# zdule/distributed_learning

Measured on AMD Instinct MI355X. Metric: images/sec (whole node) ResNet-50 synthetic ImageNet, higher is better.
Workload: dtype bf16

## Files before the change

csrc/include/dla_kernels.h:

```cpp
#pragma once

#include <hip/hip_runtime.h>
#include <stdint.h>

#include "dla_dtype.h"
#include "dla_lists.h"

namespace dla {

struct SgdParams {
  float lr;
  float momentum;
  float dampening;
  float weight_decay;
  float grad_scale;
  int nesterov;
  int first_step;
};

void launch_sgd_ema_list(const SgdList& list, const EmaSlots& ema, const float* omd, int nblocks, int grad_dtype,
                         bool use_momentum, const SgdParams& hp, hipStream_t stream);
void launch_ema_update_list(const EmaList& list, int nblocks, const float* omd, hipStream_t stream);
void launch_ema_swap_list(const EmaList& list, int nblocks, hipStream_t stream);
void launch_sgd_list(const SgdList& list, int nblocks, int grad_dtype, bool use_momentum, const SgdParams& hp,
// ... 120 lines not shown
                   int64_t M, int C, int dtype, const float* gamma, float* ws, float* part, float* dgamma,
                   float* dbeta, int mask_mode, hipStream_t stream, const float* ext_part = nullptr,
                   int ext_nrb = 0, int64_t ld_dy = 0);

constexpr int kMaxBnGroups = 4;
struct BnGroups {
  int n;
  int begin[kMaxBnGroups + 1];
  const uint16_t* x[kMaxBnGroups];
  uint16_t* y[kMaxBnGroups];
  const uint16_t* dy[kMaxBnGroups];
  int64_t ldy[kMaxBnGroups], lddy[kMaxBnGroups];
  int64_t ldx[kMaxBnGroups], lddx[kMaxBnGroups];
  int ldp[kMaxBnGroups];
  int C[kMaxBnGroups], tpr[kMaxBnGroups], nrb[kMaxBnGroups];
  const float* part[kMaxBnGroups];
  float* wpart[kMaxBnGroups];
  const float* gamma[kMaxBnGroups];
  const float* beta[kMaxBnGroups];
  float* rm[kMaxBnGroups];
  float* rv[kMaxBnGroups];
  float* ws[kMaxBnGroups];
  float eps[kMaxBnGroups], mom[kMaxBnGroups];
  uint16_t* dx[kMaxBnGroups];
  float* dgamma[kMaxBnGroups];
  float* dbeta[kMaxBnGroups];
};
int bn_group_bwd_rows(int64_t M, const int* C, int n);
void launch_bn_group_fwd(BnGroups G, int64_t M, hipStream_t stream);
void launch_bn_group_bwd(BnGroups G, bool ext, int64_t M, hipStream_t stream);

void launch_bn_relu_maxpool_fwd(const void* x, const float* ws, void* y, uint8_t* pos, int N, int H, int W, int C,
                                int OH, int OW, int k, int s, int p, hipStream_t stream);
void launch_bn_relu_maxpool_bwd(const void* dy_pool, const uint8_t* pos, const void* x, void* dx, int N, int H, int W,
                                int C, int OH, int OW, int k, int s, int p, const float* gamma, float* ws, float* part,
                                float* dgamma, float* dbeta, hipStream_t stream);

void launch_maxpool_fwd(const void* x, void* y, uint8_t* pos, int N, int H, int W, int C, int OH, int OW, int k,
                        int s, int p, int dtype, hipStream_t stream);
void launch_maxpool_bwd(const void* dy, const uint8_t* pos, void* dx, int N, int H, int W, int C, int OH, int OW,
                        int k, int s, int p, int dtype, hipStream_t stream);
bool pool_fast_index(int64_t work, int64_t d0, int64_t d1, int64_t d2);
void set_pool3_sep(int rows);
int pool3_strip_rows();
void launch_gap_fwd(const void* x, void* y, int N, int HW, int C, int dtype, hipStream_t stream);
void launch_subsample2(const void* x, void* y, int N, int H, int W, int C, hipStream_t stream);
void launch_gap_bwd(const void* dy, void* dx, int N, int HW, int C, int dtype, hipStream_t stream);

void set_mfma_pipeline(int p);
int mfma_pipeline();
int mfma_pipeline_for(int K);
enum TileCfg : int {
  kTileAuto = 0,
  kTile128x128 = 1,
  kTile128x64 = 2,
  kTile64x64 = 3,
  kTile256x128 = 4,
  kTile256x128w4 = 5,
  kTile128x256w4 = 6,
  kTile256x64 = 7,
  kTile256x256 = 8,
  kTile512x128 = 9
};
int pick_tile(int64_t M, int N, int tile, int K = 0, bool wide_ok = true, bool stats = false);
void set_tile256_min_k_stats(int k);
bool tile256_enabled();
bool tn256_enabled();
inline int tile_bm(int cfg) {
  if (cfg == kTile512x128) return 512;
  return cfg == kTile64x64 ? 64
                           : ((cfg == kTile256x128 || cfg == kTile256x128w4 || cfg == kTile256x64 || cfg == kTile256x256)
                                  ? 256
                                  : 128);
}
inline int tile_bn(int cfg) {
  if (cfg == kTile512x128) return 128;
  return (cfg == kTile128x256w4 || cfg == kTile256x256) ? 256
                                                       : ((cfg == kTile128x128 || cfg == kTile256x128 || cfg == kTile256x128w4) ? 128 : 64);
}
int gemm_nt_stats_rows(int M, int N, int tile = kTileAuto, int K = 0, bool stats_fwd = true);
void set_tile256_min_k(int k);
int gemm_stream_rows(int64_t M, int N, int K, int64_t lda, int64_t ldc, bool b_kmajor, bool add = false,
                     bool bnb = false);
struct BnBwdArgs;
bool launch_gemm_stream(const void* A, int64_t lda, const void* B, int64_t ldb, bool b_kmajor, void* C, int64_t ldc,
                        int M, int N, int K, float* stats, hipStream_t stream, const void* addend = nullptr,
                        int64_t ldd = 0, const uint8_t* addend_mask = nullptr, const BnBwdArgs* bn_bwd = nullptr,
                        const float* apply_ws = nullptr, void* apply_out = nullptr);
void set_gemm_stream(int mode);
bool gemm_direct_ok(int N, int64_t ldc, const void* addend, int64_t ldd);
void launch_gemm_direct(const void* A, int64_t lda, const void* B, int64_t ldb, bool b_kmajor, void* C, int64_t ldc,
                        int M, int N, int K, float* stats, const void* addend, int64_t ldd,
                        const uint8_t* addend_mask, hipStream_t stream);
void set_gemm_direct(int mode);
constexpr int kGemmApplyMaxK = 2048;
bool gemm_apply_ok(int64_t M, int N, int K);
void set_gemm_apply_max_k(int k);
void set_gemm256_direct(int mode);
bool gemm256_direct_enabled();
void set_wgrad_w4(int mode);
int gemm_apply_rows(int64_t M);
void launch_gemm_apply(const void* y, const void* r, const float* ws, const float* ws2, void* out, uint8_t* mask,
                       const void* B, int64_t ldb, void* C, int M, int N, int K, float* stats, hipStream_t stream,
                       void* xs = nullptr, int H = 0, int W = 0);
void set_gemm_persist(int blocks_per_cu);
bool conv_f32_supported(int C, int Cout, int64_t M, int K);
bool conv_f32_divisors_ok(int OH, int OW, int C, int S);
void set_conv_f32_buffers(int nb);
void launch_conv_f32_fwd(const float* x, int64_t ldx, int N, int H, int W, int C, const float* w, int Cout, int R,
                         int S, int pad, int stride, float* y, bool accumulate, hipStream_t st);
int conv_f32_wgrad_splits(int64_t M, int Cout, int K);
void launch_conv_f32_wgrad(const float* dy, const float* x, int64_t ldx, int N, int H, int W, int C, int Cout, int R,
                           int S, int pad, int stride, float* partial, int splits, float* dw, bool accumulate,
                           hipStream_t st);
struct BnBwdArgs {
  const void* x;
  const float* ws;
  const uint8_t* mask;
  int mode;
  float* part;
  int64_t ldx = 0;
};
void launch_gemm_nt(const void* A, int64_t lda, const void* B, int64_t ldb, void* C, int64_t ldc, int M, int N, int K,
                    float* stats, hipStream_t stream, const void* addend = nullptr, int64_t ld_addend = 0,
                    bool b_kmajor = false, int tile = kTileAuto, const BnBwdArgs* bn_bwd = nullptr,
                    const uint8_t* addend_mask = nullptr,
                    const void* addend2_s2 = nullptr, int H = 0, int W = 0);
int gemm_tn_splits(int Mo, int No, int K);
bool splitk_xcd_remap();
void set_tn256(int mode);
void set_splitk_blocks(int blocks);
int splitk_target_blocks();
void launch_gemm_tn(const void* A, int64_t lda, const void* B, int64_t ldb, float* partial, int splits, int Mo, int No,
                    int K, void* out, int out_dtype, float scale, bool accumulate, hipStream_t stream);
int conv1x1_dual_blocks(int64_t M, int Cin, int Cout);
int conv1x1_dual_groups(int64_t M, int Cin, int Cout);
bool conv1x1_dual_bn_ok(int64_t M, int Cin, int Cout);
bool launch_conv1x1_dual(const void* dy, const void* x, const void* w, void* dx, float* part, int64_t M, int Cin,
                         int Cout, hipStream_t stream, const void* ybn = nullptr, const uint8_t* mask = nullptr,
                         const float* ws = nullptr);
void launch_splitk_reduce(const float* partial, int splits, int64_t n, void* out, int out_dtype, float scale,
                          bool accumulate, hipStream_t stream, const void* addend = nullptr, int64_t ld_addend = 0,
                          int ncol = 1);
int gemm_nt_splitk_splits(int M, int N, int K);
void launch_gemm_nt_splitk(const void* A, int64_t lda, const void* B, int64_t ldb, bool b_kmajor, float* partial,
                           int splits, void* C, int M, int N, int K, const void* addend, int64_t ld_addend,
                           hipStream_t stream);

int conv3x3_stats_rows(int64_t P, int Cout, int tile = kTileAuto, int K = 0, bool wide_ok = true);
int pick_conv_tile(int64_t P, int N, int tile, int K, bool wide_ok);
bool halo_conv_eligible(int Cin, int Cout, int W, int stride, bool fwd);
void launch_conv3x3_halo(const void* x, const void* w, void* y, int N, int H, int W, float* stats,
                         hipStream_t stream, const void* addend = nullptr);
void launch_conv3x3_fwd(const void* x, const void* w, void* y, int N, int H, int W, int Cin, int Cout, int stride,
                        float* stats, hipStream_t stream, int tile = kTileAuto);
void launch_conv3x3_dgrad(const void* dy, const void* w, void* dx, int N, int H, int W, int Cin, int Cout,
                          const void* addend, hipStream_t stream, int tile = kTileAuto,
                          const BnBwdArgs* bn_bwd = nullptr);
void launch_conv3x3s2_dgrad(const void* dy, const void* w, void* dx, int N, int H, int W, int Cin, int Cout,
                            hipStream_t stream);
int stem_stats_rows(int64_t P, int Cout = 64);
int stem_stream_rows(int64_t P, int Cout);
bool launch_stem_stream(const void* xs, const void* wpk, void* y, int N, int BH, int BW, float* stats,
                        hipStream_t stream);
void set_stem_stream(int mode);

// ... 23 lines not shown
```

csrc/kernels/gemm_stream.hip:

```cpp
#include <cstdlib>

#include "dla_common.h"
#include "dla_kernels.h"
#include "dla_knob.h"
#include "dla_mfma.h"

namespace dla {

using namespace mm;

namespace {

constexpr int kSBM = 128;
constexpr int kChunkElems = kSBM * kBK;
__host__ __device__ constexpr int stream_lookahead(int KC, bool add) { return add ? 2 : 4; }

struct StreamArgs {
  const bf16_t* a;
  int64_t lda;
  const bf16_t* b;
  int64_t ldb;
  bf16_t* c;
  int64_t ldc;
  int M, N;
  int mg;
  int per_xcd;
  float* stats;
  const bf16_t* d;
  int64_t ldd;
  const uint8_t* dmask;
  const bf16_t* bx;
  int64_t ldbx;
  const float* bws;
  const uint8_t* bmask;
  int bmode;
  const float* aws;
  bf16_t* aout;
  int sBH, sBW;
  FastDiv sfW, sfH;
  uint32_t a_bytes;
};

__device__ __forceinline__ int perm64(int p) { return 16 * ((p >> 2) & 3) + 4 * (p >> 4) + (p & 3); }

__device__ __forceinline__ int img_off(int row, int lc) { return row * kBK + ((lc ^ ((row >> 1) & 7)) << 3); }

typedef int i32x4_t __attribute__((ext_vector_type(4)));


__host__ __device__ constexpr bool stream_two_blocks(bool add, bool bnb) { return add && !bnb; }

template <int BN, int KC, bool kBT, bool kStats, bool kAdd = false, int kBM = -1, bool kAp = false,
          bool kStem = false>
__global__ __launch_bounds__(256, stream_two_blocks(kAdd, kBM >= 0) ? 2 : 1) void gemm_stream_kernel(const StreamArgs s) {
  constexpr bool kBnb = kBM >= 0;
  static_assert(!kStem || (!kBT && !kAdd && !kBnb && !kAp && KC == 4), "stem: the K = 256 forward");
  static_assert(!kAp || (!kBT && !kAdd && !kBnb), "apply-on-load: forwards only");
  static_assert(!(kStats && kBnb), "the partials buffer holds either the statistics or the BN-backward sums");
  constexpr int kSP = stream_lookahead(KC, stream_two_blocks(kAdd, kBnb));
  constexpr int kSS = kSP + 1;
  constexpr int WN = 64;
  constexpr int WGN = BN / WN;
  constexpr int WGM = 4 / WGN;
  constexpr int WM = kSBM / WGM;
  constexpr int TJ = WM / 16;
  constexpr int Q = kSP / KC;
  static_assert(kSP % KC == 0, "the in-flight window must hold whole tiles");
  constexpr int D = kChunkElems / 8 / 256;
  constexpr int E = 2 * TJ;
  constexpr int F = (kAdd ? 3 * TJ : 0) + (kBnb ? (kBM == 2 ? 3 : 2) * TJ : 0);
  constexpr int kVmRaw = (kSP - 1) * (kAp ? 2 * D : D) + Q * (E + F);
  constexpr int kVmAfter = kVmRaw < 63 ? kVmRaw : 63;
  static_assert(kBnb || kVmRaw <= 63, "vmcnt is a 6-bit count");
  constexpr int kPanelElems = BN * kBK;

  extern __shared__ __attribute__((aligned(16))) char smem_raw[];
  bf16_t* Bs = reinterpret_cast<bf16_t*>(smem_raw);
  bf16_t* ring = Bs + KC * kPanelElems;
  float* coef = reinterpret_cast<float*>(ring + kSS * kChunkElems);

  const int tid = threadIdx.x, lane = tid & 63, wave = tid >> 6;
  const int wn = wave % WGN, wm = wave / WGN;
  const int lr = lane & 15, g = lane >> 4;
  const int nbn = s.N / BN;
  const int xcd = blockIdx.x & 7, slot = blockIdx.x >> 3;
  const int bn = slot % nbn;
  const int grp = xcd * s.per_xcd + slot / nbn;
  const int col0 = bn * BN;
  const int M = s.M;
  const int mt = (M + kSBM - 1) / kSBM;
  const int ntile = grp < mt ? (mt - grp + s.mg - 1) / s.mg : 0;
  const int nchunk = ntile * KC;

  {
    constexpr int kPer = BN * KC * kBK / 8 / 256;
    static_assert(BN * KC * kBK / 8 % 256 == 0, "whole chunks per thread");
    ushort8_t v[kPer];
#pragma unroll
    for (int u = 0; u < kPer; ++u) {
      const int c = tid + u * 256;
      if constexpr (!kBT) {
        const int n = c / (KC * 8), kc = c % (KC * 8);
        v[u] = *reinterpret_cast<const ushort8_t*>(s.b + (int64_t)(col0 + n) * s.ldb + kc * 8);
      } else {
        const int k = c / (BN / 8), nc = (c % (BN / 8)) * 8;
        v[u] = *reinterpret_cast<const ushort8_t*>(s.b + (int64_t)k * s.ldb + col0 + nc);
      }
    }
#pragma unroll
    for (int u = 0; u < kPer; ++u) {
      const int c = tid + u * 256;
      if constexpr (!kBT) {
        const int n = c / (KC * 8), kc = c % (KC * 8);
        const int row = (n & ~63) + perm64(n & 63);
        *reinterpret_cast<ushort8_t*>(Bs + (kc >> 3) * kPanelElems + img_off(row, kc & 7)) = v[u];
      } else {
        const int k = c / (BN / 8), nc = (c % (BN / 8)) * 8;
        bf16_t* sub = Bs + (k >> 6) * kPanelElems;
        const int kk = k & 63;
#pragma unroll
        for (int e = 0; e < 8; ++e) {
          const int n = nc + e, row = (n & ~63) + perm64(n & 63);
          sub[img_off(row, kk >> 3) + (kk & 7)] = v[u][e];
        }
      }
    }
  }

  const __amdgpu_buffer_rsrc_t ra = make_srd(s.a, kStem ? s.a_bytes : (uint32_t)((int64_t)M * s.lda * 2));
  int sbase[kStem ? D : 1];
  uint32_t smsk[kStem ? D : 1];
  const int stw = rm_glds_kc(tid) >> 4, shalf = rm_glds_kc(tid) & 8;
  uint32_t vo[D];
  int vr[D];
#pragma unroll
  for (int i = 0; i < D; ++i) {
    const int c = tid + i * 256, r = c >> 3;
    vr[i] = r;
    vo[i] = (uint32_t)(((int64_t)r * s.lda + rm_glds_kc(c)) * 2);
  }
  const uint32_t ring0 = lds_addr(ring) + (uint32_t)__builtin_amdgcn_readfirstlane(wave * 64 * 16);
  auto issue = [&](int q) {
    const int t = q / KC, kc = q % KC;
    const int64_t row0 = (int64_t)(grp + t * s.mg) * kSBM;
    uint32_t o[D];
    uint32_t soff;
    if constexpr (kStem) {
      if (kc == 0) {
#pragma unroll
        for (int i = 0; i < D; ++i) {
          const int64_t p = row0 + vr[i];
          smsk[i] = 0u;
          sbase[i] = 0;
          if (p < M) {
            const uint32_t q2 = fdiv((uint32_t)p, s.sfW);
            const int ow = (int)p - (int)q2 * s.sBW;
            const uint32_t nn = fdiv(q2, s.sfH);
            const int oh = (int)q2 - (int)nn * s.sBH;
            const int bw = ow - 2 + stw;
            if ((unsigned)bw < (unsigned)s.sBW) {
#pragma unroll
              for (int th = 0; th < 4; ++th) smsk[i] |= ((unsigned)(oh - 2 + th) < (unsigned)s.sBH) ? (1u << th) : 0u;
              sbase[i] = (((int)nn * s.sBH + oh - 2) * s.sBW + bw) * 16 + shalf;
            }
          }
        }
      }
#pragma unroll
      for (int i = 0; i < D; ++i)
        o[i] = ((smsk[i] >> kc) & 1u) ? (uint32_t)(sbase[i] + kc * s.sBW * 16) * 2u : kOOB;
      soff = 0u;
    } else {
#pragma unroll
      for (int i = 0; i < D; ++i) o[i] = row0 + vr[i] < M ? vo[i] : kOOB;
      soff = row0 < M ? (uint32_t)((row0 * s.lda + kc * kBK) * 2) : 0u;
    }
    bglds<D, 256 * 16>(o, ra, (uint32_t)__builtin_amdgcn_readfirstlane(soff),
                       ring0 + (uint32_t)((q % kSS) * kChunkElems * 2));
  };

  if constexpr (kAp) {
    for (int i = tid; i < 2 * KC * kBK; i += 256) coef[i] = s.aws[2 * KC * kBK + i];
  }
  asm volatile("s_waitcnt vmcnt(0) lgkmcnt(0)" ::: "memory");
  __syncthreads();

  const __amdgpu_buffer_rsrc_t rd = make_srd(kAdd ? (const void*)s.d : (const void*)s.c, kAdd ? (uint32_t)((int64_t)M * s.ldd * 2) : 0u);
  const __amdgpu_buffer_rsrc_t rmk =
      make_srd(kAdd && s.dmask ? (const void*)s.dmask : (const void*)s.c, kAdd && s.dmask ? (uint32_t)(((int64_t)M * s.ldd + 7) / 8) : 0u);
  i32x4_t dv[kAdd ? TJ : 1][2];
  uint32_t mb[kAdd ? TJ : 1];
  const __amdgpu_buffer_rsrc_t rbx = make_srd(kBnb ? (const void*)s.bx : (const void*)s.c,
                                              kBnb ? (uint32_t)((int64_t)M * s.ldbx * 2) : 0u);
  const __amdgpu_buffer_rsrc_t rbm = make_srd(kBM == 2 ? (const void*)s.bmask : (const void*)s.c,
                                              kBM == 2 ? (uint32_t)(((int64_t)M * s.ldc + 7) / 8) : 0u);
  i32x4_t xv[kBnb ? TJ : 1][2];
  uint32_t xb[kBM == 2 ? TJ : 1];
  float bmean[kBnb ? 16 : 1], bsc[kBM == 1 ? 16 : 1], bsh[kBM == 1 ? 16 : 1];
  if constexpr (kBnb) {
    const int gc = col0 + wn * WN + 16 * g;
#pragma unroll
    for (int e = 0; e < 16; ++e) {
      bmean[e] = s.bws[gc + e];
      if constexpr (kBM == 1) {
        bsc[e] = s.bws[2 * s.N + gc + e];
        bsh[e] = s.bws[3 * s.N + gc + e];
      }
    }
  }
  auto load_operands = [&](int t) {
    const int64_t row0 = (int64_t)(grp + t * s.mg) * kSBM;
    const int gc = col0 + wn * WN + 16 * g;
    if constexpr (kAdd) {
#pragma unroll
      for (int j = 0; j < TJ; ++j) {
        const int64_t gm = row0 + wm * WM + 16 * j + lr;
        const bool ok = gm < M;
        const uint32_t off = ok ? (uint32_t)((gm * s.ldd + gc) * 2) : kOOB;
        dv[j][0] = __builtin_amdgcn_raw_buffer_load_b128(rd, off, 0, 0);
        dv[j][1] = __builtin_amdgcn_raw_buffer_load_b128(rd, ok ? off + 16 : kOOB, 0, 0);
        mb[j] = __builtin_amdgcn_raw_buffer_load_b16(rmk, ok ? (uint32_t)((gm * s.ldd + gc) >> 3) : kOOB, 0, 0);
      }
    }
    if constexpr (kBnb) {
#pragma unroll
      for (int j = 0; j < TJ; ++j) {
        const int64_t gm = row0 + wm * WM + 16 * j + lr;
        const bool ok = gm < M;
        const uint32_t off = ok ? (uint32_t)((gm * s.ldbx + gc) * 2) : kOOB;
        xv[j][0] = __builtin_amdgcn_raw_buffer_load_b128(rbx, off, 0, 0);
        xv[j][1] = __builtin_amdgcn_raw_buffer_load_b128(rbx, ok ? off + 16 : kOOB, 0, 0);
        if constexpr (kBM == 2)
          xb[j] = __builtin_amdgcn_raw_buffer_load_b16(rbm, ok ? (uint32_t)((gm * s.ldc + gc) >> 3) : kOOB, 0, 0);
      }
    }
  };
#pragma unroll
  for (int q = 0; q < kSP; ++q) issue(q);

  const __amdgpu_buffer_rsrc_t rc = make_srd(s.c, (uint32_t)((int64_t)M * s.ldc * 2));
  const __amdgpu_buffer_rsrc_t rao = make_srd(kAp ? (void*)s.aout : (void*)s.c,
                                              kAp ? (uint32_t)((int64_t)M * s.lda * 2) : 0u);
  const int alk = rm_glds_kc(tid);
  const bool awriter = bn == 0;
  float st_s[4][4], st_q[4][4];
#pragma unroll
  for (int i = 0; i < 4; ++i)
#pragma unroll
    for (int r = 0; r < 4; ++r) st_s[i][r] = st_q[i][r] = 0.f;
  accv_t acc[4][TJ];

  for (int q = 0; q < nchunk; ++q) {
    if (q < kSP) vm_wait<(kSP - 1) * D>();
    else vm_wait<kVmAfter>();
    if constexpr (kAp) {
      const int kc = q % KC;
      const int64_t arow0 = (int64_t)(grp + (q / KC) * s.mg) * kSBM;
      bf16_t* slot = ring + (q % kSS) * kChunkElems;
      float sc[8], sh[8];
#pragma unroll
      for (int j = 0; j < 8; ++j) {
        sc[j] = coef[kc * kBK + alk + j];
        sh[j] = coef[KC * kBK + kc * kBK + alk + j];
      }
#pragma unroll
      for (int i = 0; i < D; ++i) {
        const int c = tid + i * 256;
        const int64_t gr = arow0 + vr[i];
        const ushort8_t v = *reinterpret_cast<const ushort8_t*>(slot + c * 8);
        ushort8_t o;
#pragma unroll
        for (int j = 0; j < 8; ++j) o[j] = gr < M ? f32_to_bf16(fmaxf(fmaf(bf16_to_f32(v[j]), sc[j], sh[j]), 0.f)) : 0;
        *reinterpret_cast<ushort8_t*>(slot + c * 8) = o;
        const uint32_t off = (awriter && gr < M) ? (uint32_t)((gr * s.lda + kc * kBK + alk) * 2) : kOOB;
        __builtin_amdgcn_raw_buffer_store_b128(__builtin_bit_cast(i32x4_t, o), rao, off, 0, 0);
      }
    }
    asm volatile("s_waitcnt lgkmcnt(0)" ::: "memory");
    __builtin_amdgcn_s_barrier();
    asm volatile("" ::: "memory");
    issue(q + kSP);
    const int kc = q % KC;
    if (kc == 0) {
#pragma unroll
      for (int i = 0; i < 4; ++i)
#pragma unroll
        for (int j = 0; j < TJ; ++j) acc[i][j] = accv_t{};
    }
    const bf16_t* As = ring + (q % kSS) * kChunkElems;
    const bf16_t* Ws = Bs + kc * kPanelElems;
#pragma unroll
    for (int kk = 0; kk < kBK / 32; ++kk) {
      bf16x8_t wf[4], xf[TJ];
#pragma unroll
      for (int i = 0; i < 4; ++i) wf[i] = rm_glds_frag(Ws, wn * WN + 16 * i, kk);
#pragma unroll
      for (int j = 0; j < TJ; ++j) xf[j] = rm_glds_frag(As, wm * WM + 16 * j, kk);
      __builtin_amdgcn_s_setprio(1);
#pragma unroll
      for (int i = 0; i < 4; ++i)
#pragma unroll
        for (int j = 0; j < TJ; ++j) acc[i][j] = mfma(wf[i], xf[j], acc[i][j]);
      __builtin_amdgcn_s_setprio(0);
    }
    if (kc == KC - 1) {
      const int64_t row0 = (int64_t)(grp + (q / KC) * s.mg) * kSBM;
      const int gc = col0 + wn * WN + 16 * g;
      load_operands(q / KC);
#pragma unroll
      for (int j = 0; j < TJ; ++j) {
        const int64_t gm = row0 + wm * WM + 16 * j + lr;
        const bool ok = gm < M;
        uint32_t w[8];
#pragma unroll
        for (int i = 0; i < 4; ++i) {
          bf16_t h[4];
#pragma unroll
          for (int r = 0; r < 4; ++r) {
            h[r] = f32_to_bf16(acc[i][j][r]);
            if constexpr (kAdd) {
              const int e = 4 * i + r;
              const uint32_t dw = (uint32_t)dv[j][e >> 3][(e >> 1) & 3];
              const float d = bf16_to_f32((bf16_t)((e & 1) ? (dw >> 16) : (dw & 0xffffu)));
              const uint32_t bits = s.dmask ? mb[j] : 0xffffu;
              h[r] = f32_to_bf16(bf16_to_f32(h[r]) + (((bits >> e) & 1u) ? d : 0.f));
            }
            if constexpr (kStats) {
              const float v = bf16_to_f32(h[r]);
              st_s[i][r] += v;
              st_q[i][r] = fmaf(v, v, st_q[i][r]);
            }
            if constexpr (kBnb) {
              const int e = 4 * i + r;
              const uint32_t xw = (uint32_t)xv[j][e >> 3][(e >> 1) & 3];
              const float xf = bf16_to_f32((bf16_t)((e & 1) ? (xw >> 16) : (xw & 0xffffu)));
              float gv = bf16_to_f32(h[r]);
              if constexpr (kBM == 1) gv = fmaf(xf, bsc[e], bsh[e]) > 0.f ? gv : 0.f;
              if constexpr (kBM == 2) gv = ((xb[j] >> e) & 1u) ? gv : 0.f;
              st_s[i][r] += gv;
              st_q[i][r] = fmaf(gv, xf - bmean[e], st_q[i][r]);
            }
          }
          w[2 * i] = (uint32_t)h[0] | ((uint32_t)h[1] << 16);
          w[2 * i + 1] = (uint32_t)h[2] | ((uint32_t)h[3] << 16);
        }
        const uint32_t off = ok ? (uint32_t)((gm * s.ldc + gc) * 2) : kOOB;
        const i32x4_t lo{(int)w[0], (int)w[1], (int)w[2], (int)w[3]};
        const i32x4_t hi{(int)w[4], (int)w[5], (int)w[6], (int)w[7]};
        __builtin_amdgcn_raw_buffer_store_b128(lo, rc, ok ? off : kOOB, 0, 0);
        __builtin_amdgcn_raw_buffer_store_b128(hi, rc, ok ? off + 16 : kOOB, 0, 0);
      }
    }
  }
  vm_wait<0>();
  if constexpr (kStats || kBnb) {
#pragma unroll
    for (int i = 0; i < 4; ++i)
#pragma unroll
      for (int r = 0; r < 4; ++r)
#pragma unroll
        for (int x = 1; x < 16; x <<= 1) {
          st_s[i][r] += __shfl_xor(st_s[i][r], x, 64);
          st_q[i][r] += __shfl_xor(st_q[i][r], x, 64);
        }
    __syncthreads();
    float* red = reinterpret_cast<float*>(smem_raw);
    if (lr == 0) {
#pragma unroll
      for (int i = 0; i < 4; ++i)
#pragma unroll
        for (int r = 0; r < 4; ++r) {
          const int n = wn * WN + 16 * g + 4 * i + r;
          red[(wm * BN + n) * 2 + 0] = st_s[i][r];
          red[(wm * BN + n) * 2 + 1] = st_q[i][r];
        }
    }
    __syncthreads();
    if (tid < BN * 2 && grp < s.mg) {
      float v = 0.f;
#pragma unroll
      for (int w = 0; w < WGM; ++w) v += red[w * BN * 2 + tid];
      s.stats[((int64_t)grp * s.N + col0) * 2 + tid] = v;
    }
  }
}

template <int BN, int KC, bool kTwo, bool kAp = false>
constexpr size_t stream_lds_bytes() {
  return (size_t)(KC * BN * kBK + (stream_lookahead(KC, kTwo) + 1) * kChunkElems) * sizeof(bf16_t) +
         (kAp ? (size_t)2 * KC * kBK * sizeof(float) : 0);
}

Knob k_gemm_stream = Knob::on_unless_0("GEMM_STREAM");
bool stream_enabled() { return k_gemm_stream.on(); }
bool stream_forced() { return k_gemm_stream.overridden() && k_gemm_stream.on(); }

struct StreamPlan {
  int bn = 0, mg = 0, per_xcd = 0, grid = 0;
};

StreamPlan stream_geometry(int64_t M, int N, bool add, bool bnb);

StreamPlan stream_plan(int64_t M, int N, int K, int64_t lda, int64_t ldc, bool b_kmajor, bool add = false,
                       bool bnb = false) {
  StreamPlan p;
  if (add && K > 128) return p;
  if (!stream_enabled() || M <= 0) return p;
  if (K != 64 && K != 128 && !(K == 256 && (b_kmajor || stream_forced()))) return p;
  if (N % 64 != 0 || lda % 8 != 0 || ldc % 8 != 0) return p;
  if (M * lda * 2 >= (int64_t)kOOB || M * ldc * 2 >= (int64_t)kOOB) return p;
  return stream_geometry(M, N, add, bnb);
}

StreamPlan stream_geometry(int64_t M, int N, bool add, bool bnb) {
  StreamPlan p;
  p.bn = N % 128 == 0 ? 128 : 64;
  const int nbn = N / p.bn;
  const int mt = (int)((M + kSBM - 1) / kSBM);
  int per_xcd = std::max(1, (stream_two_blocks(add, bnb) ? 64 : 32) / nbn);
  while (per_xcd > 1 && mt < 2 * 8 * per_xcd) per_xcd >>= 1;
  if (mt < 2 * 8 * per_xcd) return StreamPlan{};
  p.per_xcd = per_xcd;
  p.mg = 8 * per_xcd;
  p.grid = p.mg * nbn;
  return p;
}

Knob k_stem_stream = Knob::off_unless_1("STEM_STREAM");
bool stem_stream_enabled() { return k_stem_stream.on(); }

template <int BN, int KC>
void launch_stream_kc(const StreamArgs& a, int grid, bool kmajor, bool stats, bool add, hipStream_t stream) {
  const dim3 g(grid), b(256);
  if (a.aws) {
    hipLaunchKernelGGL((gemm_stream_kernel<BN, KC, false, true, false, -1, true>), g, b,
                       (stream_lds_bytes<BN, KC, false, true>()), stream, a);
    return;
  }
  const int bm = a.bx != nullptr ? a.bmode : -1;
#define DLA_SBN(ADD_, M_)                                                                                         \
  hipLaunchKernelGGL((gemm_stream_kernel<BN, KC, true, false, ADD_, M_>), g, b,                                  \
                     (stream_lds_bytes<BN, KC, stream_two_blocks(ADD_, (M_) >= 0)>()), stream, a)
  if constexpr (KC <= 2) {
    if (add) {
      switch (bm) {
        case 0: DLA_SBN(true, 0); break;
        case 1: DLA_SBN(true, 1); break;
        case 2: DLA_SBN(true, 2); break;
        default: DLA_SBN(true, -1); break;
      }
      return;
    }
  }
  if (bm >= 0) {
    switch (bm) {
      case 0: DLA_SBN(false, 0); break;
      case 1: DLA_SBN(false, 1); break;
      default: DLA_SBN(false, 2); break;
    }
    return;
  }
#undef DLA_SBN
  constexpr size_t lds = stream_lds_bytes<BN, KC, false>();
  if (kmajor) {
    if (stats) hipLaunchKernelGGL((gemm_stream_kernel<BN, KC, true, true>), g, b, lds, stream, a);
    else hipLaunchKernelGGL((gemm_stream_kernel<BN, KC, true, false>), g, b, lds, stream, a);
  } else {
    if (stats) hipLaunchKernelGGL((gemm_stream_kernel<BN, KC, false, true>), g, b, lds, stream, a);
    else hipLaunchKernelGGL((gemm_stream_kernel<BN, KC, false, false>), g, b, lds, stream, a);
  }
}

}

void set_gemm_stream(int mode) { k_gemm_stream.set(mode); }
void set_stem_stream(int mode) { k_stem_stream.set(mode); }

int stem_stream_rows(int64_t P, int Cout) {
  if (!stem_stream_enabled() || Cout != 64 || P <= 0 || P >= (1 << 24)) return 0;
  return stream_geometry(P, 64, false, false).mg;
}

bool launch_stem_stream(const void* xs, const void* wpk, void* y, int N, int BH, int BW, float* stats,
                        hipStream_t stream) {
  const int64_t P = (int64_t)N * BH * BW;
  const StreamPlan p = stream_geometry(P, 64, false, false);
  if (!stats || stem_stream_rows(P, 64) != p.mg || !p.mg) return false;
  if (BH >= (1 << 16) || BW >= (1 << 16)) return false;
  const int64_t xs_bytes = P * 16 * 2;
  if (xs_bytes >= (int64_t)kOOB || P * 64 * 2 >= (int64_t)kOOB) return false;
  StreamArgs a{};
  a.a = (const bf16_t*)xs;
  a.lda = 256;
  a.b = (const bf16_t*)wpk;
  a.ldb = 256;
  a.c = (bf16_t*)y;
  a.ldc = 64;
  a.M = (int)P;
  a.N = 64;
  a.mg = p.mg;
  a.per_xcd = p.per_xcd;
  a.stats = stats;
  a.sBH = BH;
  a.sBW = BW;
  a.sfW = make_fastdiv((uint32_t)BW);
  a.sfH = make_fastdiv((uint32_t)BH);
  a.a_bytes = (uint32_t)xs_bytes;
  hipLaunchKernelGGL((gemm_stream_kernel<64, 4, false, true, false, -1, false, true>), dim3(p.grid), dim3(256),
                     (stream_lds_bytes<64, 4, false>()), stream, a);
  return true;
}

int gemm_stream_rows(int64_t M, int N, int K, int64_t lda, int64_t ldc, bool b_kmajor, bool add, bool bnb) {
  return stream_plan(M, N, K, lda, ldc, b_kmajor, add, bnb).mg;
}

bool launch_gemm_stream(const void* A, int64_t lda, const void* B, int64_t ldb, bool b_kmajor, void* C, int64_t ldc,
                        int M, int N, int K, float* stats, hipStream_t stream, const void* addend, int64_t ldd,
                        const uint8_t* addend_mask, const BnBwdArgs* bn_bwd, const float* apply_ws,
                        void* apply_out) {
  const StreamPlan p = stream_plan(M, N, K, lda, ldc, b_kmajor, addend != nullptr, bn_bwd != nullptr);
  if (!p.mg) return false;
  if (apply_ws && (b_kmajor || !stats || addend || bn_bwd || !apply_out)) return false;
  if (addend && (stats || !b_kmajor || ldd % 8 != 0 || (int64_t)M * ldd * 2 >= (int64_t)kOOB)) return false;
  if (bn_bwd) {
    const int64_t ldbx = bn_bwd->ldx ? bn_bwd->ldx : ldc;
    if (stats || !b_kmajor || ldbx % 8 != 0 || (int64_t)M * ldbx * 2 >= (int64_t)kOOB) return false;
  }
  StreamArgs a{(const bf16_t*)A, lda, (const bf16_t*)B, ldb, (bf16_t*)C, ldc, M, N, p.mg, p.per_xcd,
               bn_bwd ? bn_bwd->part : stats, (const bf16_t*)addend, ldd, addend_mask,
               bn_bwd ? (const bf16_t*)bn_bwd->x : nullptr, bn_bwd ? (bn_bwd->ldx ? bn_bwd->ldx : ldc) : 0,
               bn_bwd ? bn_bwd->ws : nullptr, bn_bwd ? bn_bwd->mask : nullptr, bn_bwd ? bn_bwd->mode : 0,
               apply_ws, (bf16_t*)apply_out};
  const int kc = K / kBK;
  if (p.bn == 128) {
    if (kc == 1) launch_stream_kc<128, 1>(a, p.grid, b_kmajor, stats != nullptr, addend != nullptr, stream);
    else if (kc == 2) launch_stream_kc<128, 2>(a, p.grid, b_kmajor, stats != nullptr, addend != nullptr, stream);
    else launch_stream_kc<128, 4>(a, p.grid, b_kmajor, stats != nullptr, addend != nullptr, stream);
  } else {
    if (kc == 1) launch_stream_kc<64, 1>(a, p.grid, b_kmajor, stats != nullptr, addend != nullptr, stream);
    else if (kc == 2) launch_stream_kc<64, 2>(a, p.grid, b_kmajor, stats != nullptr, addend != nullptr, stream);
    else launch_stream_kc<64, 4>(a, p.grid, b_kmajor, stats != nullptr, addend != nullptr, stream);
  }
  return true;
}

}
```

csrc/nn_bindings.cpp:

```cpp
#include <torch/extension.h>
#include <ATen/hip/HIPContext.h>
#include <c10/hip/HIPStream.h>

#include "dla_bindings.h"
#include "dla_kernels.h"
#include "dla_knob.h"
#include "dla_tables.h"

namespace dla {

static void check_span(const at::Tensor& t, const char* what) {
  int64_t last = 0;
  for (int64_t d = 0; d < t.dim(); ++d) last += (t.size(d) - 1) * t.stride(d);
  const int64_t bytes = t.numel() ? (last + 1) * (int64_t)t.element_size() : 0;
  TORCH_CHECK(bytes < (int64_t(1) << 31), what, ": ", bytes,
              " bytes reach the 2 GiB buffer-descriptor range of the native kernels (lower the per-GPU batch)");
}

static void check_act(const at::Tensor& t, const char* what) {
  TORCH_CHECK(t.is_cuda(), what, " must be a GPU tensor");
  TORCH_CHECK(t.dim() == 4 || t.dim() == 2, what, " must be NCHW-shaped (channels_last) or [M, C]");
  const bool ok = t.dim() == 4 ? t.is_contiguous(at::MemoryFormat::ChannelsLast) : t.is_contiguous();
  TORCH_CHECK(ok, what, " must be channels_last (4-D) or contiguous (2-D)");
  TORCH_CHECK(t.size(1) % 8 == 0, what, ": channel count must be a multiple of 8");
// ... 1018 lines not shown
  TORCH_CHECK(Cout % 64 == 0 || tile_bm(tile) * tile_bn(tile) <= 128 * 128,
              "conv3x3_dgrad: Cout % 64 != 0 needs a tile of at most 128x128");
  const void* add = dgrad_addend("conv3x3_dgrad", addend, dx);
  if (tile == 0 && halo_conv_eligible(Cout, Cin, W, 1, false)) {
    const at::Tensor wt = w.flip({2, 3}).transpose(0, 1).contiguous(at::MemoryFormat::ChannelsLast);
    launch_conv3x3_halo(dy.data_ptr(), wt.data_ptr(), dx.data_ptr(), N, H, W, nullptr, current_stream(dy), add);
    return dx;
  }
  launch_conv3x3_dgrad(dy.data_ptr(), w.data_ptr(), dx.data_ptr(), N, H, W, Cin, Cout, add, current_stream(dy),
                       (int)tile);
  return dx;
}

at::Tensor conv3x3s2_dgrad(at::Tensor dy, at::Tensor w, int64_t H, int64_t W) {
  TORCH_CHECK(dy.dim() == 4 && H > 0 && W > 0 && H % 2 == 0 && W % 2 == 0 && dy.size(2) == H / 2 && dy.size(3) == W / 2,
              "conv3x3s2_dgrad: needs even H, W and dy = [N, Cout, H/2, W/2]");
  at::Tensor dx = dgrad_dx("conv3x3s2_dgrad", dy, w, H, W);
  const int N = (int)dy.size(0), Cout = (int)w.size(0), Cin = (int)w.size(1);
  TORCH_CHECK(Cin % 64 == 0 && Cout % 64 == 0, "conv3x3s2_dgrad: Cin and Cout must be multiples of 64");
  launch_conv3x3s2_dgrad(dy.data_ptr(), w.data_ptr(), dx.data_ptr(), N, (int)H, (int)W, Cin, Cout,
                         current_stream(dy));
  return dx;
}

std::vector<at::Tensor> conv3x3_dgrad_bn(at::Tensor dy, at::Tensor w, c10::optional<at::Tensor> addend,
                                         at::Tensor x_bn, at::Tensor ws, c10::optional<at::Tensor> mask, int64_t mode) {
  at::Tensor dx = dgrad_dx("conv3x3_dgrad_bn", dy, w);
  const int N = (int)dy.size(0), Cout = (int)w.size(0), Cin = (int)w.size(1), H = (int)dy.size(2), W = (int)dy.size(3);
  const void* add = dgrad_addend("conv3x3_dgrad_bn", addend, dx);
  const int64_t P = (int64_t)N * H * W;
  at::Tensor part;
  const BnBwdArgs bnb = make_bn_bwd("conv3x3_dgrad_bn", x_bn, ws, mask, mode, P, Cin,
                                    conv3x3_stats_rows(P, Cin, kTileAuto, 9 * Cout, Cout % 64 == 0), part);
  launch_conv3x3_dgrad(dy.data_ptr(), w.data_ptr(), dx.data_ptr(), N, H, W, Cin, Cout, add, current_stream(dy),
                       kTileAuto, &bnb);
  return {dx, part};
}

at::Tensor conv3x3_wgrad(at::Tensor dy, at::Tensor x, int64_t stride, c10::ScalarType out_dtype) {
  const int out_code = out_dtype_code(out_dtype, "conv3x3_wgrad");
  dy = dy.contiguous(at::MemoryFormat::ChannelsLast);
  TORCH_CHECK(x.is_cuda() && x.dim() == 4 && x.scalar_type() == at::kBFloat16 &&
                  x.is_contiguous(at::MemoryFormat::ChannelsLast) && x.size(1) % 8 == 0,
              "conv3x3_wgrad: x must be bf16 channels_last with Cin % 8 == 0");
  TORCH_CHECK(dy.is_cuda() && dy.scalar_type() == at::kBFloat16 && dy.size(1) % 8 == 0,
              "conv3x3_wgrad: dy must be a bf16 GPU tensor, Cout % 8");
  TORCH_CHECK(x.numel() / x.size(1) < (1 << 24), "conv3x3_wgrad: too many pixels");
  TORCH_CHECK(x.size(2) < 65536 && x.size(3) < 65536, "conv3x3_wgrad: H and W must be below 65536");
  check_span(x, "conv3x3_wgrad x");
  check_span(dy, "conv3x3_wgrad dy");
  const int N = (int)x.size(0), Cin = (int)x.size(1), H = (int)x.size(2), W = (int)x.size(3), Cout = (int)dy.size(1);
  TORCH_CHECK(dy.size(2) == (H - 1) / stride + 1 && dy.size(3) == (W - 1) / stride + 1, "conv3x3_wgrad: dy shape");
  at::Tensor dw = at::empty({Cout, Cin, 3, 3}, x.options().dtype(out_dtype).memory_format(at::MemoryFormat::ChannelsLast));
  if (halo_wgrad_serves(N, H, W, Cin, Cout, (int)stride)) {
    const int hs = halo_wgrad_splits(N, H, W);
    at::Tensor hpart = at::empty({(int64_t)hs * Cout * 9 * Cin}, x.options().dtype(at::kFloat));
    launch_conv3x3_halo_wgrad(dy.data_ptr(), x.data_ptr(), hpart.data_ptr<float>(), hs, dw.data_ptr(), out_code, N, H, W,
                              current_stream(x));
    return dw;
  }
  const int splits = conv3x3_wgrad_splits(N, H, W, Cin, Cout, (int)stride);
  at::Tensor part = at::empty({(int64_t)splits * Cout * 9 * Cin}, x.options().dtype(at::kFloat));
  launch_conv3x3_wgrad(dy.data_ptr(), x.data_ptr(), part.data_ptr<float>(), splits, dw.data_ptr(), out_code, N, H, W,
                       Cin, Cout, (int)stride, current_stream(x));
  return dw;
}

void bind_nn(pybind11::module& m) {
  m.def("gemm_nt_bn", &gemm_nt_bn, "gemm_nt producing a fused BN's dy plus its backward-reduction partials",
        pybind11::arg("A"), pybind11::arg("B"), pybind11::arg("addend"), pybind11::arg("b_kmajor"),
        pybind11::arg("x_bn"), pybind11::arg("ws"), pybind11::arg("mask"), pybind11::arg("mode"),
        pybind11::arg("addend_mask") = pybind11::none(), pybind11::arg("addend2") = pybind11::none(),
        pybind11::arg("H") = 0, pybind11::arg("W") = 0);
  m.def("conv3x3_dgrad_bn", &conv3x3_dgrad_bn, "3x3 dgrad producing a fused BN's dy plus its backward partials",
        pybind11::arg("dy"), pybind11::arg("w"), pybind11::arg("addend"), pybind11::arg("x_bn"), pybind11::arg("ws"),
        pybind11::arg("mask"), pybind11::arg("mode"));
  m.def("set_mfma_pipeline", &set_mfma_pipeline, "MFMA main loop: 0 register staging, 2/3 LDS-DMA stages, -1 per-shape auto");
  m.def("set_gemm_stream", &set_gemm_stream, "persistent streaming 1x1 GEMM: -1 environment (default on), 0 off, 1 on");
  m.def("set_gemm_persist", &set_gemm_persist, "persistent register-stored 1x1 GEMM: blocks per CU (0 off, -1 env)");
  m.def("set_gemm_direct", &set_gemm_direct, "register-stored 128x128 1x1 GEMM tiles: -1 environment (default off), 0 / 1");
  m.def("gemm_stream_rows", &gemm_stream_rows, "BN-statistics partial rows of the streaming GEMM (0: shape not served)",
        pybind11::arg("M"), pybind11::arg("N"), pybind11::arg("K"), pybind11::arg("lda"), pybind11::arg("ldc"), pybind11::arg("b_kmajor") = false,
        pybind11::arg("add") = false, pybind11::arg("bnb") = false);
  m.def("mfma_pipeline", &mfma_pipeline);
  m.def("set_tile256_min_k_stats", &set_tile256_min_k_stats, "smallest K of the auto 256x256 tiles of statistics forwards (A/B)");
  m.def("set_tile256_min_k", &set_tile256_min_k, "smallest K of the auto 256x256 gemm_nt / conv tiles (A/B; <= 0 default 1024)");
  m.def("set_tn256", &set_tn256, "256x256 weight-gradient tiles: -1 environment (DLA_TN256, default on), 0 off, 1 on");
  m.def("set_splitk_blocks", &set_splitk_blocks, "split-K weight-gradient block target (0 = default / DLA_SPLITK_BLOCKS)");
  m.def("splitk_target_blocks", &splitk_target_blocks);
  m.def("set_bn_red_blocks", &set_bn_red_blocks, "BN reduction-pass block target (0 = default / DLA_BN_RED_BLOCKS)");
  m.def("bn_red_blocks", &bn_red_blocks);
  m.def("conv3x3_fwd", &conv3x3_fwd, "implicit-GEMM 3x3/pad-1 conv forward (NHWC bf16, MFMA)", pybind11::arg("x"),
        pybind11::arg("w"), pybind11::arg("stride") = 1, pybind11::arg("stats") = false, pybind11::arg("tile") = 0);
  m.def("conv3x3_dgrad", &conv3x3_dgrad, "implicit-GEMM 3x3 conv data gradient (stride 1)", pybind11::arg("dy"),
        pybind11::arg("w"), pybind11::arg("addend") = pybind11::none(), pybind11::arg("tile") = 0);
  m.def("conv3x3s2_dgrad", &conv3x3s2_dgrad, "implicit-GEMM 3x3 / stride-2 conv data gradient (parity classes)",
        pybind11::arg("dy"), pybind11::arg("w"), pybind11::arg("H"), pybind11::arg("W"));
  m.def("conv3x3_wgrad", &conv3x3_wgrad, "implicit-GEMM 3x3 conv weight gradient (split-K)", pybind11::arg("dy"),
        pybind11::arg("x"), pybind11::arg("stride") = 1, pybind11::arg("out_dtype") = at::kFloat);
  m.def("bn_relu_maxpool_fwd", &bn_relu_maxpool_fwd, "stem BN(train)+ReLU+max-pool forward (pooled output only)",
        pybind11::arg("x"), pybind11::arg("weight"), pybind11::arg("bias"), pybind11::arg("running_mean"),
        pybind11::arg("running_var"), pybind11::arg("momentum"), pybind11::arg("eps"), pybind11::arg("k"),
        pybind11::arg("s"), pybind11::arg("p"), pybind11::arg("stats") = pybind11::none(),
        pybind11::arg("ceil_mode") = false);
  m.def("bn_relu_maxpool_bwd", &bn_relu_maxpool_bwd, "stem BN+ReLU+max-pool backward (dy gathered from the pool)",
        pybind11::arg("dy_pool"), pybind11::arg("pos"), pybind11::arg("x"), pybind11::arg("ws"), pybind11::arg("weight"),
        pybind11::arg("k"), pybind11::arg("s"), pybind11::arg("p"), pybind11::arg("want_dx") = true);
  m.def("maxpool_fwd", &maxpool_fwd, "NHWC max pooling forward (+ argmax window positions)", pybind11::arg("x"),
        pybind11::arg("k"), pybind11::arg("s"), pybind11::arg("p"), pybind11::arg("ceil_mode") = false,
        pybind11::arg("need_pos") = true);
  m.def("maxpool_bwd", &maxpool_bwd, "NHWC max pooling backward (gather form)");
  m.def("set_pool3_sep", &set_pool3_sep, "3x3/s1 max-pool forward: 4 / 7-row separable strips, 0 generic kernel, -1 environment (default 4)");
  m.def("pool3_strip_rows", &pool3_strip_rows, "strip height of the 3x3/s1 max-pool forward in force (0: generic kernel)");
  m.def("pool_fast_index", &pool_fast_index, "whether a pool kernel over `work` indices with divisors d0, d1, d2 decodes by multiply-shift",
        pybind11::arg("work"), pybind11::arg("d0"), pybind11::arg("d1"), pybind11::arg("d2"));
  m.def("bn_dual_fwd", &bn_dual_fwd, "training act(BN(x) + BN_d(xd)) in one apply pass (downsample residual)",
        pybind11::arg("x"), pybind11::arg("xd"), pybind11::arg("weight"), pybind11::arg("bias"),
        pybind11::arg("running_mean"), pybind11::arg("running_var"), pybind11::arg("weight_d"), pybind11::arg("bias_d"),
        pybind11::arg("running_mean_d"), pybind11::arg("running_var_d"), pybind11::arg("momentum"),
        pybind11::arg("momentum_d"), pybind11::arg("eps"), pybind11::arg("eps_d"), pybind11::arg("relu"),
        pybind11::arg("stats"), pybind11::arg("stats_d"), pybind11::arg("defer") = false);
  m.def("bn_apply_deferred", &bn_apply_deferred, "the apply pass of a deferred bn_act_fwd / bn_dual_fwd (ReLU, residual)",
        pybind11::arg("x"), pybind11::arg("r"), pybind11::arg("ws"), pybind11::arg("wsd"), pybind11::arg("y"),
        pybind11::arg("mask"));
  m.def("gemm_nt_apply", &gemm_nt_apply,
        "1x1-conv forward over a deferred act(BN(y) + r): writes the BN output + mask and returns (C, stats)",
        pybind11::arg("y"), pybind11::arg("r"), pybind11::arg("ws"), pybind11::arg("wsd"), pybind11::arg("B"),
        pybind11::arg("stats"), pybind11::arg("out"), pybind11::arg("mask"), pybind11::arg("xs") = pybind11::none(),
        pybind11::arg("H") = 0, pybind11::arg("W") = 0);
  m.def("gemm_nt_apply_ok", &gemm_nt_apply_ok, "shapes gemm_nt_apply serves (M rows, N outputs, K channels)");
  m.def("gemm_nt_stream_apply", &gemm_nt_stream_apply,
        "streaming 1x1-conv forward over a deferred BN+ReLU output: writes relu(BN(y)) and returns (C, stats)",
        pybind11::arg("y"), pybind11::arg("ws"), pybind11::arg("B"), pybind11::arg("out"));
  m.def("gemm_nt_stream_apply_ok", &gemm_nt_stream_apply_ok, "shapes gemm_nt_stream_apply serves (M, N, K)");
  m.def("set_gemm256_direct", &set_gemm256_direct, "256x256 statistics forwards stored from registers (-1 env, 0, 1)");
  m.def("set_stem_stream", &set_stem_stream, "stem forward on the persistent streaming GEMM (-1 env, 0, 1)");
  m.def("set_wgrad_w4", &set_wgrad_w4, "128x256 tiles for the Cout-128 3x3 weight gradients (-1 env, 0, 1)");
  m.def("set_gemm_apply_max_k", &set_gemm_apply_max_k, "largest K gemm_nt_apply serves (<= 0: environment / 512)");
  m.def("bn_dual_bwd", &bn_dual_bwd, "backward of bn_dual_fwd (one dy read for both BatchNorms)", pybind11::arg("dy"),
        pybind11::arg("mask"), pybind11::arg("x"), pybind11::arg("ws"), pybind11::arg("weight"), pybind11::arg("xd"),
        pybind11::arg("wsd"), pybind11::arg("weight_d"), pybind11::arg("want_dx") = true);
  m.def("gap_fwd", &gap_fwd, "NHWC global average pooling -> [N, C]");
  m.def("subsample2", &subsample2, "x[:, :, ::2, ::2] of a channels_last bf16 tensor, compact channels_last");
  m.def("stem_fwd", &stem_fwd, "7x7/s2/p3 stem conv, 3 input channels (space-to-depth + MFMA implicit GEMM, BN-statistics epilogue)");
  m.def("stem_wgrad_bn", &stem_wgrad_bn,
        "stem weight gradient with the BN+ReLU+max-pool backward apply fused (the conv-output gradient never stored)");
  m.def("stem_wgrad_bn_splits", [](int64_t N, int64_t H, int64_t W) { return stem_wgrad_bn_splits((int)N, (int)H, (int)W); },
        "split count stem_wgrad_bn uses for a batch of N images of H x W");
  m.def("stem_wgrad", &stem_wgrad, "7x7/s2/p3 stem conv weight gradient from the folded input (packed [Cout, 256] layout)");
  m.def("gap_bwd", &gap_bwd, "NHWC global average pooling backward (channels_last dx)");
  m.def("gemm_nt", &gemm_nt, "C = A @ B^T (bf16 MFMA), optional fused column statistics", pybind11::arg("A"),
        pybind11::arg("B"), pybind11::arg("stats") = false, pybind11::arg("addend") = pybind11::none(),
        pybind11::arg("b_kmajor") = false, pybind11::arg("tile") = 0,
        pybind11::arg("addend_mask") = pybind11::none(), pybind11::arg("addend2") = pybind11::none(),
        pybind11::arg("H") = 0, pybind11::arg("W") = 0);
  m.def("gemm_nt_splitk_splits", [](int64_t M, int64_t N, int64_t K) { return gemm_nt_splitk_splits((int)M, (int)N, (int)K); },
        "split count gemm_nt uses for this shape (1 = tile kernel)");
  m.def("pick_tile", [](int64_t M, int64_t N, int64_t K, bool wide_ok, bool stats) {
        return pick_tile(M, (int)N, kTileAuto, (int)K, wide_ok, stats); },
        "tile config the auto policy picks for an M x N GEMM with reduction K (TileCfg: 1 = 128x128, 2 = 128x64, 8 = 256x256); "
        "stats: a forward with the BN-statistics epilogue and no addend",
        pybind11::arg("M"), pybind11::arg("N"), pybind11::arg("K"), pybind11::arg("wide_ok"), pybind11::arg("stats") = false);
  m.def("pick_conv_tile", [](int64_t P, int64_t N, int64_t K, bool wide_ok) { return pick_conv_tile(P, (int)N, kTileAuto, (int)K, wide_ok); },
        "tile of a 3x3 forward / data-gradient launch (pick_tile + the conv-only 512x128 tile)");
  m.def("gemm_tn_splits", [](int64_t Mo, int64_t No, int64_t K) { return gemm_tn_splits((int)Mo, (int)No, (int)K); },
        "split-K count of a weight-gradient gemm_tn launch");
// ... 48 lines not shown
```

Measured before the change: 15810.

## Run K=128 statistics forward streaming GEMM at two blocks per CU

Adds a two-block-per-CU variant of the persistent streaming 1x1 GEMM for K=128 forwards with BN statistics. It shortens the lookahead ring from 4 to 2 chunks and doubles the per-XCD grid. In the apply-on-load variant it keeps the scale/shift coefficients in registers instead of LDS, which frees LDS so two blocks can fit. The variant is on by default and is meant to hide memory latency through occupancy rather than deep prefetch. The cost is a shallower pipeline per block and higher register pressure under launch_bounds(256,2), which may cause spills.

Measured after the change: 15870 (median of 6 runs). Within noise of the previous version (+0.3%).

```diff
diff --git a/csrc/include/dla_kernels.h b/csrc/include/dla_kernels.h
--- a/csrc/include/dla_kernels.h
+++ b/csrc/include/dla_kernels.h
@@ -226,6 +226,8 @@
 void set_tile256_min_k(int k);
 int gemm_stream_rows(int64_t M, int N, int K, int64_t lda, int64_t ldc, bool b_kmajor, bool add = false,
                      bool bnb = false);
+void set_stream_fwd2(int mode);
+int stream_fwd2_occupancy(int bn, bool apply);
 struct BnBwdArgs;
 bool launch_gemm_stream(const void* A, int64_t lda, const void* B, int64_t ldb, bool b_kmajor, void* C, int64_t ldc,
                         int M, int N, int K, float* stats, hipStream_t stream, const void* addend = nullptr,
diff --git a/csrc/kernels/gemm_stream.hip b/csrc/kernels/gemm_stream.hip
--- a/csrc/kernels/gemm_stream.hip
+++ b/csrc/kernels/gemm_stream.hip
@@ -13,7 +13,7 @@
 
 constexpr int kSBM = 128;
 constexpr int kChunkElems = kSBM * kBK;
-__host__ __device__ constexpr int stream_lookahead(int KC, bool add) { return add ? 2 : 4; }
+__host__ __device__ constexpr int stream_lookahead(int KC, bool two) { return two ? 2 : 4; }
 
 struct StreamArgs {
   const bf16_t* a;
@@ -48,16 +48,23 @@
 typedef int i32x4_t __attribute__((ext_vector_type(4)));
 
 
-__host__ __device__ constexpr bool stream_two_blocks(bool add, bool bnb) { return add && !bnb; }
+__host__ __device__ constexpr bool stream_two_blocks(bool add, bool bnb, bool fwd2 = false) {
+  return (add && !bnb) || fwd2;
+}
+__host__ __device__ constexpr bool stream_fwd2_shape(int KC, bool bt, bool stats, bool add, bool bnb) {
+  return KC == 2 && !bt && stats && !add && !bnb;
+}
 
 template <int BN, int KC, bool kBT, bool kStats, bool kAdd = false, int kBM = -1, bool kAp = false,
-          bool kStem = false>
-__global__ __launch_bounds__(256, stream_two_blocks(kAdd, kBM >= 0) ? 2 : 1) void gemm_stream_kernel(const StreamArgs s) {
+          bool kStem = false, bool kFwd2 = false>
+__global__ __launch_bounds__(256, stream_two_blocks(kAdd, kBM >= 0, kFwd2) ? 2 : 1) void gemm_stream_kernel(const StreamArgs s) {
   constexpr bool kBnb = kBM >= 0;
+  static_assert(!kFwd2 || (stream_fwd2_shape(KC, kBT, kStats, kAdd, kBnb) && !kStem),
+                "two-block forward: K = 128 with statistics only");
   static_assert(!kStem || (!kBT && !kAdd && !kBnb && !kAp && KC == 4), "stem: the K = 256 forward");
   static_assert(!kAp || (!kBT && !kAdd && !kBnb), "apply-on-load: forwards only");
   static_assert(!(kStats && kBnb), "the partials buffer holds either the statistics or the BN-backward sums");
-  constexpr int kSP = stream_lookahead(KC, stream_two_blocks(kAdd, kBnb));
+  constexpr int kSP = stream_lookahead(KC, stream_two_blocks(kAdd, kBnb, kFwd2));
   constexpr int kSS = kSP + 1;
   constexpr int WN = 64;
   constexpr int WGN = BN / WN;
@@ -78,6 +85,8 @@
   bf16_t* Bs = reinterpret_cast<bf16_t*>(smem_raw);
   bf16_t* ring = Bs + KC * kPanelElems;
   float* coef = reinterpret_cast<float*>(ring + kSS * kChunkElems);
+  constexpr bool kCoefReg = kAp && kFwd2;
+  float csc0[8], csh0[8], csc1[8], csh1[8];
 
   const int tid = threadIdx.x, lane = tid & 63, wave = tid >> 6;
   const int wn = wave % WGN, wm = wave / WGN;
@@ -179,7 +188,16 @@
                        ring0 + (uint32_t)((q % kSS) * kChunkElems * 2));
   };
 
-  if constexpr (kAp) {
+  if constexpr (kCoefReg) {
+    const int ak = rm_glds_kc(tid);
+#pragma unroll
+    for (int j = 0; j < 8; ++j) {
+      csc0[j] = s.aws[2 * KC * kBK + ak + j];
+      csc1[j] = s.aws[2 * KC * kBK + kBK + ak + j];
+      csh0[j] = s.aws[3 * KC * kBK + ak + j];
+      csh1[j] = s.aws[3 * KC * kBK + kBK + ak + j];
+    }
+  } else if constexpr (kAp) {
     for (int i = tid; i < 2 * KC * kBK; i += 256) coef[i] = s.aws[2 * KC * kBK + i];
   }
   asm volatile("s_waitcnt vmcnt(0) lgkmcnt(0)" ::: "memory");
@@ -260,8 +278,13 @@
       float sc[8], sh[8];
 #pragma unroll
       for (int j = 0; j < 8; ++j) {
-        sc[j] = coef[kc * kBK + alk + j];
-        sh[j] = coef[KC * kBK + kc * kBK + alk + j];
+        if constexpr (kCoefReg) {
+          sc[j] = kc ? csc1[j] : csc0[j];
+          sh[j] = kc ? csh1[j] : csh0[j];
+        } else {
+          sc[j] = coef[kc * kBK + alk + j];
+          sh[j] = coef[KC * kBK + kc * kBK + alk + j];
+        }
       }
 #pragma unroll
       for (int i = 0; i < D; ++i) {
@@ -388,36 +411,46 @@
 template <int BN, int KC, bool kTwo, bool kAp = false>
 constexpr size_t stream_lds_bytes() {
   return (size_t)(KC * BN * kBK + (stream_lookahead(KC, kTwo) + 1) * kChunkElems) * sizeof(bf16_t) +
-         (kAp ? (size_t)2 * KC * kBK * sizeof(float) : 0);
+         (kAp && !kTwo ? (size_t)2 * KC * kBK * sizeof(float) : 0);
 }
 
 Knob k_gemm_stream = Knob::on_unless_0("GEMM_STREAM");
 bool stream_enabled() { return k_gemm_stream.on(); }
 bool stream_forced() { return k_gemm_stream.overridden() && k_gemm_stream.on(); }
 
+#ifndef DLA_STREAM_FWD2
+#define DLA_STREAM_FWD2 1
+#endif
+int g_stream_fwd2 = -1;
+bool stream_fwd2_on() { return g_stream_fwd2 < 0 ? DLA_STREAM_FWD2 != 0 : g_stream_fwd2 != 0; }
+
 struct StreamPlan {
   int bn = 0, mg = 0, per_xcd = 0, grid = 0;
+  bool fwd2 = false;
 };
 
-StreamPlan stream_geometry(int64_t M, int N, bool add, bool bnb);
+StreamPlan stream_geometry(int64_t M, int N, bool two);
 
 StreamPlan stream_plan(int64_t M, int N, int K, int64_t lda, int64_t ldc, bool b_kmajor, bool add = false,
-                       bool bnb = false) {
+                       bool bnb = false, bool fwd_stats = false) {
   StreamPlan p;
   if (add && K > 128) return p;
   if (!stream_enabled() || M <= 0) return p;
   if (K != 64 && K != 128 && !(K == 256 && (b_kmajor || stream_forced()))) return p;
   if (N % 64 != 0 || lda % 8 != 0 || ldc % 8 != 0) return p;
   if (M * lda * 2 >= (int64_t)kOOB || M * ldc * 2 >= (int64_t)kOOB) return p;
-  return stream_geometry(M, N, add, bnb);
-}
-
-StreamPlan stream_geometry(int64_t M, int N, bool add, bool bnb) {
+  const bool fwd2 = stream_fwd2_shape(K / kBK, b_kmajor, fwd_stats, add, bnb) && stream_fwd2_on();
+  p = stream_geometry(M, N, stream_two_blocks(add, bnb, fwd2));
+  p.fwd2 = fwd2 && p.mg > 0;
+  return p;
+}
+
+StreamPlan stream_geometry(int64_t M, int N, bool two) {
   StreamPlan p;
   p.bn = N % 128 == 0 ? 128 : 64;
   const int nbn = N / p.bn;
   const int mt = (int)((M + kSBM - 1) / kSBM);
-  int per_xcd = std::max(1, (stream_two_blocks(add, bnb) ? 64 : 32) / nbn);
+  int per_xcd = std::max(1, (two ? 64 : 32) / nbn);
   while (per_xcd > 1 && mt < 2 * 8 * per_xcd) per_xcd >>= 1;
   if (mt < 2 * 8 * per_xcd) return StreamPlan{};
   p.per_xcd = per_xcd;
@@ -430,9 +463,17 @@
 bool stem_stream_enabled() { return k_stem_stream.on(); }
 
 template <int BN, int KC>
-void launch_stream_kc(const StreamArgs& a, int grid, bool kmajor, bool stats, bool add, hipStream_t stream) {
+void launch_stream_kc(const StreamArgs& a, int grid, bool kmajor, bool stats, bool add, bool fwd2,
+                      hipStream_t stream) {
   const dim3 g(grid), b(256);
   if (a.aws) {
+    if constexpr (KC == 2) {
+      if (fwd2) {
+        hipLaunchKernelGGL((gemm_stream_kernel<BN, KC, false, true, false, -1, true, false, true>), g, b,
+                           (stream_lds_bytes<BN, KC, true, true>()), stream, a);
+        return;
+      }
+    }
     hipLaunchKernelGGL((gemm_stream_kernel<BN, KC, false, true, false, -1, true>), g, b,
                        (stream_lds_bytes<BN, KC, false, true>()), stream, a);
     return;
@@ -461,6 +502,13 @@
     return;
   }
 #undef DLA_SBN
+  if constexpr (KC == 2) {
+    if (fwd2) {
+      hipLaunchKernelGGL((gemm_stream_kernel<BN, KC, false, true, false, -1, false, false, true>), g, b,
+                         (stream_lds_bytes<BN, KC, true>()), stream, a);
+      return;
+    }
+  }
   constexpr size_t lds = stream_lds_bytes<BN, KC, false>();
   if (kmajor) {
     if (stats) hipLaunchKernelGGL((gemm_stream_kernel<BN, KC, true, true>), g, b, lds, stream, a);
@@ -475,16 +523,32 @@
 
 void set_gemm_stream(int mode) { k_gemm_stream.set(mode); }
 void set_stem_stream(int mode) { k_stem_stream.set(mode); }
+void set_stream_fwd2(int mode) { g_stream_fwd2 = mode < 0 ? -1 : (mode != 0); }
+
+template <int BN, bool kAp>
+int fwd2_occupancy() {
+  int blocks = 0;
+  DLA_HIP_CHECK(hipOccupancyMaxActiveBlocksPerMultiprocessor(
+      &blocks, gemm_stream_kernel<BN, 2, false, true, false, -1, kAp, false, true>, 256,
+      stream_lds_bytes<BN, 2, true, kAp>()));
+  return blocks;
+}
+
+int stream_fwd2_occupancy(int bn, bool apply) {
+  if (bn == 128) return apply ? fwd2_occupancy<128, true>() : fwd2_occupancy<128, false>();
+  if (bn == 64) return apply ? fwd2_occupancy<64, true>() : fwd2_occupancy<64, false>();
+  return 0;
+}
 
 int stem_stream_rows(int64_t P, int Cout) {
   if (!stem_stream_enabled() || Cout != 64 || P <= 0 || P >= (1 << 24)) return 0;
-  return stream_geometry(P, 64, false, false).mg;
+  return stream_geometry(P, 64, false).mg;
 }
 
 bool launch_stem_stream(const void* xs, const void* wpk, void* y, int N, int BH, int BW, float* stats,
                         hipStream_t stream) {
   const int64_t P = (int64_t)N * BH * BW;
-  const StreamPlan p = stream_geometry(P, 64, false, false);
+  const StreamPlan p = stream_geometry(P, 64, false);
   if (!stats || stem_stream_rows(P, 64) != p.mg || !p.mg) return false;
   if (BH >= (1 << 16) || BW >= (1 << 16)) return false;
   const int64_t xs_bytes = P * 16 * 2;
@@ -512,14 +576,15 @@
 }
 
 int gemm_stream_rows(int64_t M, int N, int K, int64_t lda, int64_t ldc, bool b_kmajor, bool add, bool bnb) {
-  return stream_plan(M, N, K, lda, ldc, b_kmajor, add, bnb).mg;
+  return stream_plan(M, N, K, lda, ldc, b_kmajor, add, bnb, true).mg;
 }
 
 bool launch_gemm_stream(const void* A, int64_t lda, const void* B, int64_t ldb, bool b_kmajor, void* C, int64_t ldc,
                         int M, int N, int K, float* stats, hipStream_t stream, const void* addend, int64_t ldd,
                         const uint8_t* addend_mask, const BnBwdArgs* bn_bwd, const float* apply_ws,
                         void* apply_out) {
-  const StreamPlan p = stream_plan(M, N, K, lda, ldc, b_kmajor, addend != nullptr, bn_bwd != nullptr);
+  const StreamPlan p = stream_plan(M, N, K, lda, ldc, b_kmajor, addend != nullptr, bn_bwd != nullptr,
+                                   stats != nullptr);
   if (!p.mg) return false;
   if (apply_ws && (b_kmajor || !stats || addend || bn_bwd || !apply_out)) return false;
   if (addend && (stats || !b_kmajor || ldd % 8 != 0 || (int64_t)M * ldd * 2 >= (int64_t)kOOB)) return false;
@@ -534,13 +599,13 @@
                apply_ws, (bf16_t*)apply_out};
   const int kc = K / kBK;
   if (p.bn == 128) {
-    if (kc == 1) launch_stream_kc<128, 1>(a, p.grid, b_kmajor, stats != nullptr, addend != nullptr, stream);
-    else if (kc == 2) launch_stream_kc<128, 2>(a, p.grid, b_kmajor, stats != nullptr, addend != nullptr, stream);
-    else launch_stream_kc<128, 4>(a, p.grid, b_kmajor, stats != nullptr, addend != nullptr, stream);
+    if (kc == 1) launch_stream_kc<128, 1>(a, p.grid, b_kmajor, stats != nullptr, addend != nullptr, p.fwd2, stream);
+    else if (kc == 2) launch_stream_kc<128, 2>(a, p.grid, b_kmajor, stats != nullptr, addend != nullptr, p.fwd2, stream);
+    else launch_stream_kc<128, 4>(a, p.grid, b_kmajor, stats != nullptr, addend != nullptr, p.fwd2, stream);
   } else {
-    if (kc == 1) launch_stream_kc<64, 1>(a, p.grid, b_kmajor, stats != nullptr, addend != nullptr, stream);
-    else if (kc == 2) launch_stream_kc<64, 2>(a, p.grid, b_kmajor, stats != nullptr, addend != nullptr, stream);
-    else launch_stream_kc<64, 4>(a, p.grid, b_kmajor, stats != nullptr, addend != nullptr, stream);
+    if (kc == 1) launch_stream_kc<64, 1>(a, p.grid, b_kmajor, stats != nullptr, addend != nullptr, p.fwd2, stream);
+    else if (kc == 2) launch_stream_kc<64, 2>(a, p.grid, b_kmajor, stats != nullptr, addend != nullptr, p.fwd2, stream);
+    else launch_stream_kc<64, 4>(a, p.grid, b_kmajor, stats != nullptr, addend != nullptr, p.fwd2, stream);
   }
   return true;
 }
diff --git a/csrc/nn_bindings.cpp b/csrc/nn_bindings.cpp
--- a/csrc/nn_bindings.cpp
+++ b/csrc/nn_bindings.cpp
@@ -1124,6 +1124,11 @@
   m.def("gemm_stream_rows", &gemm_stream_rows, "BN-statistics partial rows of the streaming GEMM (0: shape not served)",
         pybind11::arg("M"), pybind11::arg("N"), pybind11::arg("K"), pybind11::arg("lda"), pybind11::arg("ldc"), pybind11::arg("b_kmajor") = false,
         pybind11::arg("add") = false, pybind11::arg("bnb") = false);
+  m.def("set_stream_fwd2", &set_stream_fwd2,
+        "K = 128 streaming forwards with statistics: -1 build default (two blocks per CU), 0 one block, 1 two");
+  m.def("stream_fwd2_occupancy", &stream_fwd2_occupancy,
+        "co-resident blocks per CU of the two-block K = 128 streaming forward (bn = 128 / 64) at its launch LDS size",
+        pybind11::arg("bn"), pybind11::arg("apply") = false);
   m.def("mfma_pipeline", &mfma_pipeline);
   m.def("set_tile256_min_k_stats", &set_tile256_min_k_stats, "smallest K of the auto 256x256 tiles of statistics forwards (A/B)");
   m.def("set_tile256_min_k", &set_tile256_min_k, "smallest K of the auto 256x256 gemm_nt / conv tiles (A/B; <= 0 default 1024)");
```
